# eovs/ldpc-lib

Hardware: AMD Instinct MI355X
Metric: decoded frames/sec, (2048,1024) QC-LDPC, 50 iters min-sum (higher is better)
Workload: dtype f64

## Files before the change

ldpc-lib_amd/csrc/ldpc_spec.hpp:

```cpp
#pragma once

#ifndef __HIPCC_RTC__
#include <hip/hip_runtime.h>
#endif
#include "lche_table.hpp"

namespace ldpc_spec {

typedef unsigned int u32;
typedef unsigned long long u64;

struct SpecArgs {
    const double *llr;
    u32 *hard;
    int *iters;
    double *soft_out;
    int maxiter;
    double alpha;
    const u32 *stale;
    u32 *synd_out;
    const int *frame_idx;
    const double *ims_coef;
    double ims_thr;
    int ims_max_quant, ims_max_data, ims_ialpha;
// ... 64 lines not shown
    0x0000000000000000ull, 0x3ff0000000000000ull, 0x3c9b3b4f1a88bf6eull, 0x3feff63da9fb3335ull,
    0xbc7160139cd8dc5dull, 0x3fefec9a3e778061ull, 0xbc905e7a108766d1ull, 0x3fefe315e86e7f85ull,
    0x3c8cd2523567f613ull, 0x3fefd9b0d3158574ull, 0xbc8bce8023f98efaull, 0x3fefd06b29ddf6deull,
    0x3c60f74e61e6c861ull, 0x3fefc74518759bc8ull, 0x3c90a3e45b33d399ull, 0x3fefbe3ecac6f383ull,
    0x3c979aa65d837b6dull, 0x3fefb5586cf9890full, 0x3c8eb51a92fdeffcull, 0x3fefac922b7247f7ull,
    0x3c3ebe3d702f9cd1ull, 0x3fefa3ec32d3d1a2ull, 0xbc6a033489906e0bull, 0x3fef9b66affed31bull,
    0xbc9556522a2fbd0eull, 0x3fef9301d0125b51ull, 0xbc5080ef8c4eea55ull, 0x3fef8abdc06c31ccull,
    0xbc91c923b9d5f416ull, 0x3fef829aaea92de0ull, 0x3c80d3e3e95c55afull, 0x3fef7a98c8a58e51ull,
    0xbc801b15eaa59348ull, 0x3fef72b83c7d517bull, 0xbc8f1ff055de323dull, 0x3fef6af9388c8deaull,
    0x3c8b898c3f1353bfull, 0x3fef635beb6fcb75ull, 0xbc96d99c7611eb26ull, 0x3fef5be084045cd4ull,
    0x3c9aecf73e3a2f60ull, 0x3fef54873168b9aaull, 0xbc8fe782cb86389dull, 0x3fef4d5022fcd91dull,
    0x3c8a6f4144a6c38dull, 0x3fef463b88628cd6ull, 0x3c807a05b0e4047dull, 0x3fef3f49917ddc96ull,
    0x3c968efde3a8a894ull, 0x3fef387a6e756238ull, 0x3c875e18f274487dull, 0x3fef31ce4fb2a63full,
    0x3c80472b981fe7f2ull, 0x3fef2b4565e27cddull, 0xbc96b87b3f71085eull, 0x3fef24dfe1f56381ull,
    0x3c82f7e16d09ab31ull, 0x3fef1e9df51fdee1ull, 0xbc3d219b1a6fbffaull, 0x3fef187fd0dad990ull,
    0x3c8b3782720c0ab4ull, 0x3fef1285a6e4030bull, 0x3c6e149289cecb8full, 0x3fef0cafa93e2f56ull,
    0x3c834d754db0abb6ull, 0x3fef06fe0a31b715ull, 0x3c864201e2ac744cull, 0x3fef0170fc4cd831ull,
    0x3c8fdd395dd3f84aull, 0x3feefc08b26416ffull, 0xbc86a3803b8e5b04ull, 0x3feef6c55f929ff1ull,
    0xbc924aedcc4b5068ull, 0x3feef1a7373aa9cbull, 0xbc9907f81b512d8eull, 0x3feeecae6d05d866ull,
    0xbc71d1e83e9436d2ull, 0x3feee7db34e59ff7ull, 0xbc991919b3ce1b15ull, 0x3feee32dc313a8e5ull,
    0x3c859f48a72a4c6dull, 0x3feedea64c123422ull, 0xbc9312607a28698aull, 0x3feeda4504ac801cull,
    0xbc58a78f4817895bull, 0x3feed60a21f72e2aull, 0xbc7c2c9b67499a1bull, 0x3feed1f5d950a897ull,
    0x3c4363ed60c2ac11ull, 0x3feece086061892dull, 0x3c9666093b0664efull, 0x3feeca41ed1d0057ull,
    0x3c6ecce1daa10379ull, 0x3feec6a2b5c13cd0ull, 0x3c93ff8e3f0f1230ull, 0x3feec32af0d7d3deull,
    0x3c7690cebb7aafb0ull, 0x3feebfdad5362a27ull, 0x3c931dbdeb54e077ull, 0x3feebcb299fddd0dull,
    0xbc8f94340071a38eull, 0x3feeb9b2769d2ca7ull, 0xbc87deccdc93a349ull, 0x3feeb6daa2cf6642ull,
    0xbc78dec6bd0f385full, 0x3feeb42b569d4f82ull, 0xbc861246ec7b5cf6ull, 0x3feeb1a4ca5d920full,
    0x3c93350518fdd78eull, 0x3feeaf4736b527daull, 0x3c7b98b72f8a9b05ull, 0x3feead12d497c7fdull,
    0x3c9063e1e21c5409ull, 0x3feeab07dd485429ull, 0x3c34c7855019c6eaull, 0x3feea9268a5946b7ull,
    0x3c9432e62b64c035ull, 0x3feea76f15ad2148ull, 0xbc8ce44a6199769full, 0x3feea5e1b976dc09ull,
    0xbc8c33c53bef4da8ull, 0x3feea47eb03a5585ull, 0xbc845378892be9aeull, 0x3feea34634ccc320ull,
    0xbc93cedd78565858ull, 0x3feea23882552225ull, 0x3c5710aa807e1964ull, 0x3feea155d44ca973ull,
    0xbc93b3efbf5e2228ull, 0x3feea09e667f3bcdull, 0xbc6a12ad8734b982ull, 0x3feea012750bdabfull,
    0xbc6367efb86da9eeull, 0x3fee9fb23c651a2full, 0xbc80dc3d54e08851ull, 0x3fee9f7df9519484ull,
    0xbc781f647e5a3ecfull, 0x3fee9f75e8ec5f74ull, 0xbc86ee4ac08b7db0ull, 0x3fee9f9a48a58174ull,
    0xbc8619321e55e68aull, 0x3fee9feb564267c9ull, 0x3c909ccb5e09d4d3ull, 0x3feea0694fde5d3full,
    0xbc7b32dcb94da51dull, 0x3feea11473eb0187ull, 0x3c94ecfd5467c06bull, 0x3feea1ed0130c132ull,
    0x3c65ebe1abd66c55ull, 0x3feea2f336cf4e62ull, 0xbc88a1c52fb3cf42ull, 0x3feea427543e1a12ull,
    0xbc9369b6f13b3734ull, 0x3feea589994cce13ull, 0xbc805e843a19ff1eull, 0x3feea71a4623c7adull,
    0xbc94d450d872576eull, 0x3feea8d99b4492edull, 0x3c90ad675b0e8a00ull, 0x3feeaac7d98a6699ull,
    0x3c8db72fc1f0eab4ull, 0x3feeace5422aa0dbull, 0xbc65b6609cc5e7ffull, 0x3feeaf3216b5448cull,
    0x3c7bf68359f35f44ull, 0x3feeb1ae99157736ull, 0xbc93091fa71e3d83ull, 0x3feeb45b0b91ffc6ull,
    0xbc5da9b88b6c1e29ull, 0x3feeb737b0cdc5e5ull, 0xbc6c23f97c90b959ull, 0x3feeba44cbc8520full,
    0xbc92434322f4f9aaull, 0x3feebd829fde4e50ull, 0xbc85ca6cd7668e4bull, 0x3feec0f170ca07baull,
    0x3c71affc2b91ce27ull, 0x3feec49182a3f090ull, 0x3c6dd235e10a73bbull, 0x3feec86319e32323ull,
    0xbc87c50422622263ull, 0x3feecc667b5de565ull, 0x3c8b1c86e3e231d5ull, 0x3feed09bec4a2d33ull,
    0xbc91bbd1d3bcbb15ull, 0x3feed503b23e255dull, 0x3c90cc319cee31d2ull, 0x3feed99e1330b358ull,
    0x3c8469846e735ab3ull, 0x3feede6b5579fdbfull, 0xbc82dfcd978e9db4ull, 0x3feee36bbfd3f37aull,
    0x3c8c1a7792cb3387ull, 0x3feee89f995ad3adull, 0xbc907b8f4ad1d9faull, 0x3feeee07298db666ull,
    0xbc55c3d956dcaebaull, 0x3feef3a2b84f15fbull, 0xbc90a40e3da6f640ull, 0x3feef9728de5593aull,
    0xbc68d6f438ad9334ull, 0x3feeff76f2fb5e47ull, 0xbc91eee26b588a35ull, 0x3fef05b030a1064aull,
    0x3c74ffd70a5fddcdull, 0x3fef0c1e904bc1d2ull, 0xbc91bdfbfa9298acull, 0x3fef12c25bd71e09ull,
    0x3c736eae30af0cb3ull, 0x3fef199bdd85529cull, 0x3c8ee3325c9ffd94ull, 0x3fef20ab5fffd07aull,
    0x3c84e08fd10959acull, 0x3fef27f12e57d14bull, 0x3c63cdaf384e1a67ull, 0x3fef2f6d9406e7b5ull,
    0x3c676b2c6c921968ull, 0x3fef3720dcef9069ull, 0xbc808a1883ccb5d2ull, 0x3fef3f0b555dc3faull,
    0xbc8fad5d3ffffa6full, 0x3fef472d4a07897cull, 0xbc900dae3875a949ull, 0x3fef4f87080d89f2ull,
    0x3c74a385a63d07a7ull, 0x3fef5818dcfba487ull, 0xbc82919e2040220full, 0x3fef60e316c98398ull,
    0x3c8e5a50d5c192acull, 0x3fef69e603db3285ull, 0x3c843a59ac016b4bull, 0x3fef7321f301b460ull,
    0xbc82d52107b43e1full, 0x3fef7c97337b9b5full, 0xbc892ab93b470dc9ull, 0x3fef864614f5a129ull,
    0x3c74b604603a88d3ull, 0x3fef902ee78b3ff6ull, 0x3c83c5ec519d7271ull, 0x3fef9a51fbc74c83ull,
    0xbc8ff7128fd391f0ull, 0x3fefa4afa2a490daull, 0xbc8dae98e223747dull, 0x3fefaf482d8e67f1ull,
    0x3c8ec3bc41aa2008ull, 0x3fefba1bee615a27ull, 0x3c842b94c3a9eb32ull, 0x3fefc52b376bba97ull,
    0x3c8a64a931d185eeull, 0x3fefd0765b6e4540ull, 0xbc8e37bae43be3edull, 0x3fefdbfdad9cbe14ull,
    0x3c77893b4d91cd9dull, 0x3fefe7c1819e90d8ull, 0x3c5305c14160cc89ull, 0x3feff3c22b8f71f1ull
};
template <class Tab>
__device__ __forceinline__ double exp_glibc_t(double x, Tab T) {
    const double InvLn2N = 0x1.71547652b82fep+7, Shift = 0x1.8p52, NegLn2hiN = -0x1.62e42fefa0000p-8, NegLn2loN = -0x1.cf79abc9e3b3ap-47;
    const double C2 = 0x1.ffffffffffdbdp-2, C3 = 0x1.555555555543cp-3, C4 = 0x1.55555cf172b91p-5, C5 = 0x1.1111167a4d017p-7;
    const double z = InvLn2N * x;
    double kd = z + Shift;
    const unsigned long long ki = (unsigned long long)__double_as_longlong(kd);
    kd -= Shift;
    const double r = __fma_rn(kd, NegLn2loN, __fma_rn(kd, NegLn2hiN, x));
    const unsigned long long idx = 2 * (ki % 128);
    const ulonglong2 pair = *reinterpret_cast<const ulonglong2 *>(&T[idx]);
    const double tail = __longlong_as_double((long long)pair.x);
    const unsigned long long sbits = pair.y + (ki << (52 - 7));
    const double r2 = r * r;
    const double tmp = __fma_rn(r2 * r2, __fma_rn(r, C5, C4), __fma_rn(r2, __fma_rn(r, C3, C2), tail + r));
    const double scale = __longlong_as_double((long long)sbits);
    return __fma_rn(scale, tmp, scale);
}
__device__ __forceinline__ double exp_glibc(double x) { return exp_glibc_t(x, kExpTab); }

__device__ __attribute__((aligned(16))) const unsigned long long kLogData[274] = {
    0x3fe62e42fefa3800ull, 0x3d2ef35793c76730ull, 0xbfe0000000000001ull, 0x3fd555555551305bull,
    0xbfcfffffffeb4590ull, 0x3fc999b324f10111ull, 0xbfc55575e506c89full, 0xbfe0000000000000ull,
    0x3fd5555555555577ull, 0xbfcffffffffffdcbull, 0x3fc999999995dd0cull, 0xbfc55555556745a7ull,
    0x3fc24924a344de30ull, 0xbfbfffffa4423d65ull, 0x3fbc7184282ad6caull, 0xbfb999eb43b068ffull,
    0x3fb78182f7afd085ull, 0xbfb5521375d145cdull, 0x3ff734f0c3e0de9full, 0xbfd7cc7f79e69000ull,
    0x3ff713786a2ce91full, 0xbfd76feec20d0000ull, 0x3ff6f26008fab5a0ull, 0xbfd713e31351e000ull,
    0x3ff6d1a61f138c7dull, 0xbfd6b85b38287800ull, 0x3ff6b1490bc5b4d1ull, 0xbfd65d5590807800ull,
    0x3ff69147332f0cbaull, 0xbfd602d076180000ull, 0x3ff6719f18224223ull, 0xbfd5a8ca86909000ull,
    0x3ff6524f99a51ed9ull, 0xbfd54f4356035000ull, 0x3ff63356aa8f24c4ull, 0xbfd4f637c36b4000ull,
    0x3ff614b36b9ddc14ull, 0xbfd49da7fda85000ull, 0x3ff5f66452c65c4cull, 0xbfd445923989a800ull,
    0x3ff5d867b5912c4full, 0xbfd3edf439b0b800ull, 0x3ff5babccb5b90deull, 0xbfd396ce448f7000ull,
    0x3ff59d61f2d91a78ull, 0xbfd3401e17bda000ull, 0x3ff5805612465687ull, 0xbfd2e9e2ef468000ull,
    0x3ff56397cee76bd3ull, 0xbfd2941b3830e000ull, 0x3ff54725e2a77f93ull, 0xbfd23ec58cda8800ull,
    0x3ff52aff42064583ull, 0xbfd1e9e129279000ull, 0x3ff50f22dbb2bddfull, 0xbfd1956d2b48f800ull,
    0x3ff4f38f4734ded7ull, 0xbfd141679ab9f800ull, 0x3ff4d843cfde2840ull, 0xbfd0edd094ef9800ull,
    0x3ff4bd3ec078a3c8ull, 0xbfd09aa518db1000ull, 0x3ff4a27fc3e0258aull, 0xbfd047e65263b800ull,
    0x3ff4880524d48434ull, 0xbfcfeb224586f000ull, 0x3ff46dce1b192d0bull, 0xbfcf474a7517b000ull,
    0x3ff453d9d3391854ull, 0xbfcea4443d103000ull, 0x3ff43a2744b4845aull, 0xbfce020d44e9b000ull,
    0x3ff420b54115f8fbull, 0xbfcd60a22977f000ull, 0x3ff40782da3ef4b1ull, 0xbfccc00104959000ull,
    0x3ff3ee8f5d57fe8full, 0xbfcc202956891000ull, 0x3ff3d5d9a00b4ce9ull, 0xbfcb81178d811000ull,
    0x3ff3bd60c010c12bull, 0xbfcae2c9ccd3d000ull, 0x3ff3a5242b75dab8ull, 0xbfca45402e129000ull,
    0x3ff38d22cd9fd002ull, 0xbfc9a877681df000ull, 0x3ff3755bc5847a1cull, 0xbfc90c6d69483000ull,
    0x3ff35dce49ad36e2ull, 0xbfc87120a645c000ull, 0x3ff34679984dd440ull, 0xbfc7d68fb4143000ull,
    0x3ff32f5cceffcb24ull, 0xbfc73cb83c627000ull, 0x3ff3187775a10d49ull, 0xbfc6a39a9b376000ull,
    0x3ff301c8373e3990ull, 0xbfc60b3154b7a000ull, 0x3ff2eb4ebb95f841ull, 0xbfc5737d76243000ull,
    0x3ff2d50a0219a9d1ull, 0xbfc4dc7b8fc23000ull, 0x3ff2bef9a8b7fd2aull, 0xbfc4462c51d20000ull,
    0x3ff2a91c7a0c1babull, 0xbfc3b08abc830000ull, 0x3ff293726014b530ull, 0xbfc31b996b490000ull,
    0x3ff27dfa5757a1f5ull, 0xbfc2875490a44000ull, 0x3ff268b39b1d3bbfull, 0xbfc1f3b9f879a000ull,
    0x3ff2539d838ff5bdull, 0xbfc160c8252ca000ull, 0x3ff23eb7aac9083bull, 0xbfc0ce7f57f72000ull,
    0x3ff22a012ba940b6ull, 0xbfc03cdc49fea000ull, 0x3ff2157996cc4132ull, 0xbfbf57bdbc4b8000ull,
    0x3ff201201dd2fc9bull, 0xbfbe370896404000ull, 0x3ff1ecf4494d480bull, 0xbfbd17983ef94000ull,
    0x3ff1d8f5528f6569ull, 0xbfbbf9674ed8a000ull, 0x3ff1c52311577e7cull, 0xbfbadc79202f6000ull,
    0x3ff1b17c74cb26e9ull, 0xbfb9c0c3e7288000ull, 0x3ff19e010c2c1ab6ull, 0xbfb8a646b372c000ull,
    0x3ff18ab07bb670bdull, 0xbfb78d01b3ac0000ull, 0x3ff1778a25efbcb6ull, 0xbfb674f145380000ull,
    0x3ff1648d354c31daull, 0xbfb55e0e6d878000ull, 0x3ff151b990275fddull, 0xbfb4485cdea1e000ull,
    0x3ff13f0ea432d24cull, 0xbfb333d94d6aa000ull, 0x3ff12c8b7210f9daull, 0xbfb22079f8c56000ull,
    0x3ff11a3028ecb531ull, 0xbfb10e4698622000ull, 0x3ff107fbda8434afull, 0xbfaffa6c6ad20000ull,
    0x3ff0f5ee0f4e6bb3ull, 0xbfadda8d4a774000ull, 0x3ff0e4065d2a9fceull, 0xbfabbcece4850000ull,
    0x3ff0d244632ca521ull, 0xbfa9a1894012c000ull, 0x3ff0c0a77ce2981aull, 0xbfa788583302c000ull,
    0x3ff0af2f83c636d1ull, 0xbfa5715e67d68000ull, 0x3ff09ddb98a01339ull, 0xbfa35c8a49658000ull,
    0x3ff08cabaf52e7dfull, 0xbfa149e364154000ull, 0x3ff07b9f2f4e28fbull, 0xbf9e72c082eb8000ull,
    0x3ff06ab58c358f19ull, 0xbf9a55f152528000ull, 0x3ff059eea5ecf92cull, 0xbf963d62cf818000ull,
    0x3ff04949cdd12c90ull, 0xbf9228fb8caa0000ull, 0x3ff038c6c6f0ada9ull, 0xbf8c317b20f90000ull,
    0x3ff02865137932a9ull, 0xbf8419355daa0000ull, 0x3ff0182427ea7348ull, 0xbf781203c2ec0000ull,
    0x3ff008040614b195ull, 0xbf60040979240000ull, 0x3fefe01ff726fa1aull, 0x3f6feff384900000ull,
    0x3fefa11cc261ea74ull, 0x3f87dc41353d0000ull, 0x3fef6310b081992eull, 0x3f93cea3c4c28000ull,
    0x3fef25f63ceeadcdull, 0x3f9b9fc114890000ull, 0x3feee9c8039113e7ull, 0x3fa1b0d8ce110000ull,
    0x3feeae8078cbb1abull, 0x3fa58a5bd001c000ull, 0x3fee741aa29d0c9bull, 0x3fa95c8340d88000ull,
    0x3fee3a91830a99b5ull, 0x3fad276aef578000ull, 0x3fee01e009609a56ull, 0x3fb07598e598c000ull,
    0x3fedca01e577bb98ull, 0x3fb253f5e30d2000ull, 0x3fed92f20b7c9103ull, 0x3fb42edd8b380000ull,
    0x3fed5cac66fb5cceull, 0x3fb606598757c000ull, 0x3fed272caa5ede9dull, 0x3fb7da76356a0000ull,
    0x3fecf26e3e6b2ccdull, 0x3fb9ab434e1c6000ull, 0x3fecbe6da2a77902ull, 0x3fbb78c7bb0d6000ull,
    0x3fec8b266d37086dull, 0x3fbd431332e72000ull, 0x3fec5894bd5d5804ull, 0x3fbf0a3171de6000ull,
    0x3fec26b533bb9f8cull, 0x3fc067152b914000ull, 0x3febf583eeece73full, 0x3fc147858292b000ull,
    0x3febc4fd75db96c1ull, 0x3fc2266ecdca3000ull, 0x3feb951e0c864a28ull, 0x3fc303d7a6c55000ull,
    0x3feb65e2c5ef3e2cull, 0x3fc3dfc33c331000ull, 0x3feb374867c9888bull, 0x3fc4ba366b7a8000ull,
    0x3feb094b211d304aull, 0x3fc5933928d1f000ull, 0x3feadbe885f2ef7eull, 0x3fc66acd2418f000ull,
    0x3feaaf1d31603da2ull, 0x3fc740f8ec669000ull, 0x3fea82e63fd358a7ull, 0x3fc815c0f51af000ull,
    0x3fea5740ef09738bull, 0x3fc8e92954f68000ull, 0x3fea2c2a90ab4b27ull, 0x3fc9bb3602f84000ull,
    0x3fea01a01393f2d1ull, 0x3fca8bed1c2c0000ull, 0x3fe9d79f24db3c1bull, 0x3fcb5b515c01d000ull,
    0x3fe9ae2505c7b190ull, 0x3fcc2967ccbcc000ull, 0x3fe9852ef297ce2full, 0x3fccf635d5486000ull,
    0x3fe95cbaeea44b75ull, 0x3fcdc1bd3446c000ull, 0x3fe934c69de74838ull, 0x3fce8c01b8cfe000ull,
    0x3fe90d4f2f6752e6ull, 0x3fcf5509c0179000ull, 0x3fe8e6528effd79dull, 0x3fd00e6c121fb800ull,
    0x3fe8bfce9fcc007cull, 0x3fd071b80e93d000ull, 0x3fe899c0dabec30eull, 0x3fd0d46b9e867000ull,
    0x3fe87427aa2317fbull, 0x3fd13687334bd000ull, 0x3fe84f00acb39a08ull, 0x3fd1980d67234800ull,
    0x3fe82a49e8653e55ull, 0x3fd1f8ffe0cc8000ull, 0x3fe8060195f40260ull, 0x3fd2595fd7636800ull,
    0x3fe7e22563e0a329ull, 0x3fd2b9300914a800ull, 0x3fe7beb377dcb5adull, 0x3fd3187210436000ull,
    0x3fe79baa679725c2ull, 0x3fd377266dec1800ull, 0x3fe77907f2170657ull, 0x3fd3d54ffbaf3000ull,
    0x3fe756cadbd6130cull, 0x3fd432eee32fe000ull
};
template <class Tab>
__device__ __forceinline__ double log_glibc_t(double x, Tab T) {
    auto D = [&](int i) { return __longlong_as_double((long long)kLogData[i]); };
    unsigned long long ix = (unsigned long long)__double_as_longlong(x);
    const u32 top = (u32)(ix >> 48);
    const unsigned long long LO = 0x3fee000000000000ull , HI = 0x3ff1090000000000ull ;
    if (ix - LO < HI - LO) {
        if (ix == 0x3ff0000000000000ull) return 0.0;
        const double r = x - 1.0, r2 = r * r, r3 = r * r2;
        const double t3 = __fma_rn(r3, D(17), __fma_rn(r2, D(16), __fma_rn(r, D(15), D(14))));
        const double t2 = __fma_rn(r3, t3, __fma_rn(r2, D(13), __fma_rn(r, D(12), D(11))));
        const double t1 = __fma_rn(r3, t2, __fma_rn(r2, D(10), __fma_rn(r, D(9), D(8))));
        double w = r * 0x1p27;
        const double rhi = r + w - w, rlo = r - rhi;
        w = rhi * rhi * D(7);
        const double hi = r + w;
        double lo = r - hi + w;
        lo = __fma_rn(D(7) * rlo, rhi + r, lo);
        return __fma_rn(t1, r3, lo) + hi;
    }
    if (top - 0x0010u >= 0x7ff0u - 0x0010u) {
        if (ix * 2 == 0) return -__longlong_as_double(0x7ff0000000000000ll);
        if (ix == 0x7ff0000000000000ull) return x;
        if ((top & 0x8000u) || (top & 0x7ff0u) == 0x7ff0u) return __longlong_as_double(0x7ff8000000000000ll) ;
        ix = (unsigned long long)__double_as_longlong(x * 0x1p52);
        ix -= 52ull << 52;
    }
    const unsigned long long tmp = ix - 0x3fe6000000000000ull;
    const int i = (int)((tmp >> (52 - 7)) % 128);
    const long long k = (long long)tmp >> 52;
    const unsigned long long iz = ix - (tmp & (0xfffull << 52));
    const ulonglong2 cpair = *reinterpret_cast<const ulonglong2 *>(&T[18 + 2 * i]);
    const double invc = __longlong_as_double((long long)cpair.x), logc = __longlong_as_double((long long)cpair.y), z = __longlong_as_double((long long)iz);
    const double r = __fma_rn(z, invc, -1.0);
    const double kd = (double)k;
    const double w = __fma_rn(kd, D(0), logc);
    const double hi = w + r;
    const double lo = __fma_rn(kd, D(1), w - hi + r);
    const double r2 = r * r;
    const double p = __fma_rn(r, D(6), D(5));
    const double q = __fma_rn(r2, p, __fma_rn(r, D(4), D(3)));
    return __fma_rn(r * r2, q, __fma_rn(r2, D(2), lo)) + hi;
}
__device__ __forceinline__ double log_glibc(double x) { return log_glibc_t(x, kLogData); }
template <class Tab>
__device__ __forceinline__ double exp_glibc_wide(double x, Tab T) {
    return fabs(x) < 512.0 ? exp_glibc_t(x, T) : exp(x);
}
constexpr int kBpTabWords = 256 + 274;

__device__ __forceinline__ double at_most(double x, double hi) { return fmin(x, hi); }
__device__ __forceinline__ double at_least(double x, double lo) { return fmax(x, lo); }

template <bool QUEUED, class F>
__device__ __forceinline__ void for_each_frame(const SpecArgs &a, long long fr, F body) {
    if constexpr (!QUEUED) {
        body(fr);
    } else {
        __shared__ unsigned q_ticket;
        while (fr < a.nframes) {
            body(fr);
            if (!a.queue) break;
            __syncthreads();
            if (threadIdx.x == 0) q_ticket = atomicAdd(a.queue, 1u);
            __syncthreads();
            fr = (long long)gridDim.x + (long long)(unsigned)__builtin_amdgcn_readfirstlane((int)q_ticket);
        }
    }
}

template <int N, int T, class Pred>
__device__ __forceinline__ void pack_hard(u32 *dst, const int tid, Pred pred) {
    constexpr int G = (N + 63) / 64, HW = (N + 31) / 32;
    const int lane = tid & 63;
    for (int g = tid >> 6; g < G; g += T / 64) {
        const int v = 64 * g + lane;
        const u64 m = __ballot(v < N && pred(v < N ? v : 0));
        if (lane == 0) {
            dst[2 * g] = (u32)m;
            if (2 * g + 1 < HW) dst[2 * g + 1] = (u32)(m >> 32);
        }
    }
}


constexpr unsigned long kMsM64LdsBytes(unsigned long n) { return sizeof(double) * n + 512; }

constexpr int kMsM64LocalSpan = 3;
template <class C>
constexpr int ms_m64_slot_of(int j, int k) {
    for (int s = 0; s < C::RW[j]; ++s)
        if (C::COL[j][s] == k) return s;
    return -1;
}
template <class C>
constexpr int ms_m64_first_row(int k) {
    for (int j = 0; j < C::RH; ++j)
        if (ms_m64_slot_of<C>(j, k) >= 0) return j;
    return -1;
}
template <class C>
constexpr int ms_m64_last_row(int k) {
    for (int j = C::RH - 1; j >= 0; --j)
        if (ms_m64_slot_of<C>(j, k) >= 0) return j;
    return -1;
}
template <class C>
constexpr bool ms_m64_local_col(int k) {
    for (int j = 0; j < C::RH; ++j) {
        const int s = ms_m64_slot_of<C>(j, k);
        if (s >= 0 && C::SH[j][s] != 0) return false;
    }
    return ms_m64_first_row<C>(k) >= 0 && ms_m64_last_row<C>(k) - ms_m64_first_row<C>(k) <= kMsM64LocalSpan;
}
template <class C>
constexpr int ms_m64_local_starts(int j) {
    int n = 0;
    for (int s = 0; j < C::RH && s < C::RW[j]; ++s)
        n += ms_m64_local_col<C>(C::COL[j][s]) && ms_m64_first_row<C>(C::COL[j][s]) == j ? 1 : 0;
    return n;
}
template <class C>
constexpr int ms_m64_row_edges(int j) {
    int n = 0;
    for (int s = 0; s < C::RW[j]; ++s) n += ms_m64_local_col<C>(C::COL[j][s]) ? 0 : 1;
    return n;
}

template <class C>
constexpr int ms_m64_keep_rows(int budget) {
    int edges = 0, rows = 0;
    while (rows < C::RH && 2 * (edges + ms_m64_row_edges<C>(rows)) - 5 * (rows + 1) <= budget) edges += ms_m64_row_edges<C>(rows++);
    return rows;
}
constexpr int kMsM64KeepEdges = 68, kMsM64KeepRowsOfExample = 13;
template <class C>
constexpr int ms_m64_keep_budget() {
    constexpr int cols = C::NH < 24 ? C::NH : 24;
    constexpr int others = 5 * C::RH + 2 * cols + 2 * C::WMAX, others_example = 5 * 16 + 2 * 24 + 2 * 8;
    constexpr int cut = others > others_example ? others - others_example : 0;
    constexpr int regs = 2 * kMsM64KeepEdges - 5 * kMsM64KeepRowsOfExample;
    return regs > cut ? regs - cut : 0;
}

template <int KPCAP>
constexpr int ms_m64_prefix_rows(int kr) { return KPCAP < kr ? (KPCAP > 0 ? KPCAP : 0) : kr; }

template <class C, int KPCAP = 1 << 30>
__device__ __forceinline__ void ms_m64_body(const SpecArgs &a) {
    static_assert(C::M == 64, "ms_m64_body: one frame per wavefront needs M == 64");
    constexpr int RH = C::RH, NH = C::NH, N = C::NH * 64;
    constexpr int KR = ms_m64_keep_rows<C>(ms_m64_keep_budget<C>());
    typedef IC<ms_m64_prefix_rows<KPCAP>(KR)> KP;
    extern __shared__ double lds[];
    const int lane = threadIdx.x;
    const double alpha = a.alpha, alpha_mag = fabs(a.alpha);
    long long fr = blockIdx.x;

    const u32 lane8 = (u32)lane * 8u;
    const u32 lo = lds_addr(lds) + lane8, hi = lo + 512u;
    auto at = [&](u32 tie, auto S, auto K) -> double * {
        constexpr int c = decltype(S)::value, k = decltype(K)::value;
        static_assert(c >= 0 && c < 64 && k * 512 + c * 8 < 65536, "shift / block column out of range");
        if constexpr (c == 0) return lds_at(hi + (u32)(k * 512));
        else return lds_at(sel32_tied(hi, lo, ~0ull << (64 - c), tie) + (u32)(k * 512 + c * 8));
    };
    auto own = [&](auto K) -> double * { return lds_at(hi + (u32)(decltype(K)::value * 512)); };

  while (fr < a.nframes) {
    const double *const yrow = a.llr + fr * N + lane;
    const __amdgpu_buffer_rsrc_t ybuf = __builtin_amdgcn_make_buffer_rsrc(const_cast<double *>(a.llr + fr * N), 0, N * 8, 0x00020000);

    double m1[RH], m2[RH];
    u32 meta[RH];
    double keep[RH][C::WMAX];
    static_for<0, RH>([&](auto J) {
        constexpr int j = decltype(J)::value;
        m1[j] = 0.0; m2[j] = 0.0; meta[j] = 0u;
        if constexpr (j < KR) static_for<0, C::RW[j]>([&](auto S) { keep[j][decltype(S)::value] = 0.0; });
    });

    int res = -a.maxiter;
    for (int iter = 0; iter < a.maxiter; ++iter) {
        double y[NH];
        auto load_y = [&](auto K0, auto K1) {
            int yo = 0;
            asm volatile("" : "+v"(yo));
            static_for<decltype(K0)::value, (decltype(K1)::value < NH ? decltype(K1)::value : NH)>([&](auto K) {
                constexpr int k = decltype(K)::value;
                if constexpr (!ms_m64_local_col<C>(k)) y[k] = yrow[yo + k * 64];
            });
        };
        double yl[NH], soft_l[NH];
        auto load_yl = [&](auto JN) {
            constexpr int jn = decltype(JN)::value;
            if constexpr (ms_m64_local_starts<C>(jn) > 0) {
                u32 so = 0;
                asm volatile("" : "+s"(so));
                static_for<0, C::RW[jn]>([&](auto S) {
                    constexpr int k = C::COL[jn][decltype(S)::value];
                    if constexpr (ms_m64_local_col<C>(k) && ms_m64_first_row<C>(k) == jn) {
                        typedef u32 u32x2 __attribute__((ext_vector_type(2)));
                        const u32x2 v = __builtin_amdgcn_raw_buffer_load_b64(ybuf, (int)lane8, (int)(so + (u32)(k * 512)), 0);
                        yl[k] = mk(v.y, v.x);
                    }
                });
            }
        };
        static_for<0, RH>([&](auto J) {
            constexpr int j = decltype(J)::value;
            if constexpr (j < KR) {
                u32 tie;
                asm volatile("" : "=v"(tie));
                static_for<0, C::RW[j]>([&](auto S) {
                    constexpr int s = decltype(S)::value;
                    if constexpr (!ms_m64_local_col<C>(C::COL[j][s])) {
                        const double cv = keep[j][s];
                        double *p = at(tie, IC<C::SH[j][s]>{}, IC<C::COL[j][s]>{});
                        if constexpr (C::FIRST[j][s]) *p = cv;
                        else __hip_atomic_fetch_add(p, cv, __ATOMIC_RELAXED, __HIP_MEMORY_SCOPE_WORKGROUP);
                    }
                });
            } else {
                u32 mt = meta[j];
                asm volatile("" : "+v"(mt));
                const u32 pos = mt & 0xffu;
                u32 Wt = mt;
                static_for<0, C::RW[j]>([&](auto S) {
                    constexpr int s = decltype(S)::value;
                    if constexpr (ms_m64_local_col<C>(C::COL[j][s])) {
                        Wt = twice(Wt);
                    } else {
                        const double aa = sel64(m1[j], m2[j], lanes_eq(pos, (u32)s));
                        const double cv = signed_mag(aa, Wt);
                        Wt = twice(Wt);
                        double *p = at(mt, IC<C::SH[j][s]>{}, IC<C::COL[j][s]>{});
                        if constexpr (C::FIRST[j][s]) *p = cv;
                        else __hip_atomic_fetch_add(p, cv, __ATOMIC_RELAXED, __HIP_MEMORY_SCOPE_WORKGROUP);
                    }
                });
            }
            __builtin_amdgcn_sched_barrier(0);
        });
        load_y(IC<0>{}, IC<16>{});
        static_for<0, NH>([&](auto K) {
            constexpr int k = decltype(K)::value;
            if constexpr (k % 8 == 0 && k + 16 < NH) load_y(IC<k + 16>{}, IC<k + 24>{});
            if constexpr (!ms_m64_local_col<C>(k)) {
                double *p = own(K);
                const double pr = *p * alpha;
                *p = (y[k] + 0.0) + pr;
            }
            if constexpr (k % 8 == 7) __builtin_amdgcn_sched_barrier(0);
        });
        load_yl(IC<0>{});
        u32 failw = 0;
        static_for<0, RH>([&](auto J) {
            constexpr int j = decltype(J)::value;
            constexpr int RW = C::RW[j];
            u32 mt = meta[j];
            asm volatile("" : "+v"(mt));
            load_yl(IC<j + 1>{});
            double nm1 = kMaxVal, nm2 = kMaxVal;
            u32 npos = 0, nS = 0, sy = 0;
            double r[RW], tt_[RW];
            static_for<0, RW>([&](auto S) {
                constexpr int s = decltype(S)::value;
                constexpr int k = C::COL[j][s];
                if constexpr (!ms_m64_local_col<C>(k)) {
                    r[s] = *at(mt, IC<C::SH[j][s]>{}, IC<k>{});
                } else {
                    if constexpr (ms_m64_first_row<C>(k) == j) {
                        double acc = 0.0;
                        static_for<j, ms_m64_last_row<C>(k) + 1>([&](auto JJ) {
                            constexpr int jj = decltype(JJ)::value, ss = ms_m64_slot_of<C>(jj, k);
                            if constexpr (ss >= 0) {
                                if constexpr (jj >= KR) {
                                    const u32 m = jj == j ? mt : meta[jj];
                                    const double aa = sel64(m1[jj], m2[jj], lanes_eq(m & 0xffu, (u32)ss));
                                    keep[jj][ss] = signed_mag(aa, ss == 0 ? m : ss == 1 ? twice(m) : m << ss);
                                }
                                const double cv = keep[jj][ss];
                                if constexpr (jj == j) acc = cv;
                                else acc = acc + cv;
                            }
                        });
                        const double pr = acc * alpha;
                        soft_l[k] = (yl[k] + 0.0) + pr;
                        *own(IC<k>{}) = soft_l[k];
                    }
                    r[s] = soft_l[k];
                }
            });
            auto step = [&](auto S, double x) {
                constexpr int s = decltype(S)::value;
                const double tt = r[s] - x;
                nS = __builtin_amdgcn_alignbit(nS, hi32(tt), 31);
                const double v = fabs(tt);
                if constexpr (j < KR) tt_[s] = tt;
                if constexpr (s == 0) {
                    nm1 = fmin(v, kMaxVal);
                } else if constexpr (j < KR) {
                    nm2 = fmin(fmax(v, nm1), nm2);
                    nm1 = fmin(v, nm1);
                } else {
                    const mask64 c1 = lanes_lt(v, nm1);
                    nm2 = fmin(fmax(v, nm1), nm2);
                    npos = sel32(npos, (u32)s, c1);
                    nm1 = fmin(v, nm1);
                }
            };
            if constexpr (j < KR) {
                if constexpr (j < KP::value) {
                    double pf[RW > 1 ? RW - 1 : 1];
                    static_for<0, RW>([&](auto S) {
                        constexpr int s = decltype(S)::value;
                        sy ^= hi32(r[s]);
                        const double tt = r[s] - keep[j][s] * alpha_mag;
                        nS ^= hi32(tt);
                        tt_[s] = tt;
                        if constexpr (s == 0 && RW > 1) pf[0] = fmin(fabs(tt), kMaxVal);
                        else if constexpr (s > 0 && s < RW - 1) pf[s] = fmin(fabs(tt), pf[s - 1]);
                    });
                    double suf = kMaxVal;
                    static_for<0, RW>([&](auto S) {
                        constexpr int s = RW - 1 - decltype(S)::value;
                        double mag;
                        if constexpr (RW == 1) mag = kMaxVal;
                        else if constexpr (s == RW - 1) mag = pf[RW - 2];
                        else if constexpr (s == 0) mag = suf;
                        else mag = fmin(pf[s - 1], suf);
                        if constexpr (s > 0) suf = fmin(fabs(tt_[s]), suf);
                        keep[j][s] = signed_mag(mag, hi32(tt_[s]) ^ nS);
                    });
                } else {
                    static_for<0, RW>([&](auto S) {
                        constexpr int s = decltype(S)::value;
                        sy ^= hi32(r[s]);
                        step(S, keep[j][s] * alpha_mag);
                    });
                }
            } else {
                const u32 pos = mt & 0xffu;
                u32 Wt = mt;
                double a1 = m1[j] * alpha, a2 = m2[j] * alpha;
                asm volatile("" : "+v"(a1), "+v"(a2));
                static_for<0, RW>([&](auto S) {
                    constexpr int s = decltype(S)::value;
                    sy ^= hi32(r[s]);
                    if constexpr (ms_m64_local_col<C>(C::COL[j][s])) {
                        Wt = twice(Wt);
                        step(S, keep[j][s] * alpha_mag);
                    } else {
                        const double aa = sel64(a1, a2, lanes_eq(pos, (u32)s));
                        const double x = signed_mag(aa, Wt);
                        Wt = twice(Wt);
                        step(S, x);
                    }
                });
            }
            failw |= sy;
            asm volatile("" : "+v"(failw));
            if constexpr (j < KR) {
                if constexpr (j >= KP::value) {
                    u32 W = (nS ^ (0u - (__popc(nS) & 1u))) << (32 - RW);
                    static_for<0, RW>([&](auto S) {
                        constexpr int s = decltype(S)::value;
                        keep[j][s] = signed_mag(sel64(nm1, nm2, lanes_oeq(fabs(tt_[s]), nm1)), W);
                        W = twice(W);
                    });
                }
            } else {
                m1[j] = nm1; m2[j] = nm2; meta[j] = ((nS ^ (0u - (__popc(nS) & 1u))) << (32 - RW)) | npos;
            }
            __builtin_amdgcn_sched_barrier(0);
        });
        if (__ballot((failw >> 31) != 0) == 0ull) { res = iter + 1; break; }
    }

    if (lane == 0 && a.iters) a.iters[fr] = res;
    if (a.hard) {
        u64 mine = 0ull;
        static_for<0, NH>([&](auto K) {
            constexpr int k = decltype(K)::value;
            const u64 b = __ballot((hi32(*own(K)) >> 31) != 0);
            if (lane == k) mine = b;
        });
        if (lane < NH) reinterpret_cast<u64 *>(a.hard + fr * (N / 32))[lane] = mine;
    }
    if (a.soft_out) {
        static_for<0, NH>([&](auto K) {
            constexpr int k = decltype(K)::value;
            a.soft_out[fr * N + k * 64 + lane] = *own(K);
        });
    }
    if (!a.queue) break;
    u32 ticket = 0;
    if (lane == 0) ticket = atomicAdd(a.queue, 1u);
    fr = (long long)gridDim.x + (long long)(u32)__builtin_amdgcn_readfirstlane((int)ticket);
  }
}

template <class C>
__device__ __forceinline__ void ms_body(const SpecArgs &a) {
    constexpr int RH = C::RH, NH = C::NH, M = C::M, N = NH * M, W = (M + 63) / 64;
    constexpr bool POW2 = (M & (M - 1)) == 0;
    extern __shared__ double lds[];
    char *const ldsb = reinterpret_cast<char *>(lds);
    int *const flag = reinterpret_cast<int *>(ldsb + (size_t)N * 8);
    const int n = threadIdx.x;
    const bool valid = (M % 64 == 0) || n < M;
    const u32 n8 = (u32)(valid ? n : 0) * 8u;
    const double alpha = a.alpha;
    for_each_frame<true>(a, (long long)blockIdx.x, [&](const long long fr) {

    auto rot = [&](u32 base, auto S) -> u32 {
        constexpr int c = decltype(S)::value;
        if constexpr (c == 0) return base;
        else if constexpr (POW2) return (base + 8u * (u32)c) & (u32)(8 * M - 1);
        else { const u32 t = base + 8u * (u32)c, w = t - (u32)(8 * M); return t < w ? t : w; }
    };
    FrameVote fvote;
    if constexpr (W > 1) fvote.init(flag);
    auto vote = [&](bool fail) -> bool {
        if constexpr (W == 1) return __ballot(fail) != 0ull;
        else return fvote(fail);
    };
    const double *const yrow = a.llr + fr * N + (valid ? n : 0);

    double m1[RH], m2[RH];
    u32 meta[RH];
    static_for<0, RH>([&](auto J) { constexpr int j = decltype(J)::value; m1[j] = 0.0; m2[j] = 0.0; meta[j] = 0u; });

    int res = -a.maxiter;
    for (int iter = 0; iter < a.maxiter; ++iter) {
        double y[NH];
        int yo = 0;
        asm volatile("" : "+v"(yo));
        static_for<0, NH>([&](auto K) { constexpr int k = decltype(K)::value; y[k] = yrow[yo + k * M]; });
        static_for<0, RH>([&](auto J) {
            constexpr int j = decltype(J)::value;
            u32 mt = meta[j], nb = n8;
            asm volatile("" : "+v"(mt), "+v"(nb) :: "memory");
            const u32 pos = mt & 0xffu;
            u32 Wt = mt;
            static_for<0, C::RW[j]>([&](auto S) {
                constexpr int s = decltype(S)::value;
                const double aa = sel64(m1[j], m2[j], lanes_eq(pos, (u32)s));
                const double cv = signed_mag(aa, Wt);
                Wt = twice(Wt);
                double *p = reinterpret_cast<double *>(ldsb + rot(nb, IC<C::SH[j][s]>{}) + C::COL[j][s] * (8 * M));
                if (valid) {
                    if constexpr (C::FIRST[j][s]) *p = cv;
                    else __hip_atomic_fetch_add(p, cv, __ATOMIC_RELAXED, __HIP_MEMORY_SCOPE_WORKGROUP);
                }
            });
            if constexpr (W > 1) __syncthreads();
            else __builtin_amdgcn_sched_barrier(0);
        });
        if (valid) {
            static_for<0, NH>([&](auto K) {
                constexpr int k = decltype(K)::value;
                double *p = reinterpret_cast<double *>(ldsb + n8 + k * (8 * M));
                const double pr = *p * alpha;
                *p = (y[k] + 0.0) + pr;
                if constexpr (k % 8 == 7) __builtin_amdgcn_sched_barrier(0);
            });
        }
        if constexpr (W > 1) __syncthreads();
        u32 failw = 0;
        static_for<0, RH>([&](auto J) {
            constexpr int j = decltype(J)::value;
            constexpr int RW = C::RW[j];
            u32 mt = meta[j];
            asm volatile("" : "+v"(mt) :: "memory");
            const u32 pos = mt & 0xffu;
            u32 Wt = mt;
            double a1 = m1[j] * alpha, a2 = m2[j] * alpha;
            asm volatile("" : "+v"(a1), "+v"(a2));
            double nm1 = kMaxVal, nm2 = kMaxVal;
            u32 npos = 0, nS = 0, sy = 0;
            u32 nb = n8;
            asm volatile("" : "+v"(nb));
            double r[RW];
            static_for<0, RW>([&](auto S) {
                constexpr int s = decltype(S)::value;
                r[s] = *reinterpret_cast<const double *>(ldsb + rot(nb, IC<C::SH[j][s]>{}) + C::COL[j][s] * (8 * M));
            });
            static_for<0, RW>([&](auto S) {
                constexpr int s = decltype(S)::value;
                sy ^= hi32(r[s]);
                const double aa = sel64(a1, a2, lanes_eq(pos, (u32)s));
                const double x = signed_mag(aa, Wt);
                Wt = twice(Wt);
                const double tt = r[s] - x;
                nS = __builtin_amdgcn_alignbit(nS, hi32(tt), 31);
                const double v = fabs(tt);
                const mask64 c1 = lanes_lt(v, nm1);
                nm2 = fmin(fmax(v, nm1), nm2);
                npos = sel32(npos, (u32)s, c1);
                nm1 = fmin(v, nm1);
            });
            failw |= sy;
            m1[j] = nm1; m2[j] = nm2; meta[j] = ((nS ^ (0u - (__popc(nS) & 1u))) << (32 - RW)) | npos;
            asm volatile("" : "+v"(m1[j]), "+v"(m2[j]), "+v"(meta[j]));
            __builtin_amdgcn_sched_barrier(0);
        });
        if (!vote(valid && (failw >> 31) != 0)) { res = iter + 1; break; }
    }

    if (threadIdx.x == 0 && a.iters) a.iters[fr] = res;
    if (a.hard) {
        constexpr int HW = (N + 31) / 32;
        if constexpr (M % 64 == 0) {
            const int wave = threadIdx.x >> 6, lane = threadIdx.x & 63;
            static_for<0, NH>([&](auto K) {
                constexpr int k = decltype(K)::value;
                const u64 b = __ballot((*reinterpret_cast<const u32 *>(ldsb + n8 + k * (8 * M) + 4) >> 31) != 0);
                if (lane == 0) reinterpret_cast<u64 *>(a.hard + fr * HW)[k * W + wave] = b;
            });
        } else {
            pack_hard<N, W * 64>(a.hard + fr * HW, threadIdx.x, [&](int v) { return (*reinterpret_cast<const u32 *>(ldsb + (size_t)v * 8 + 4) >> 31) != 0; });
        }
    }
    if (a.soft_out && valid) {
        static_for<0, NH>([&](auto K) {
            constexpr int k = decltype(K)::value;
            a.soft_out[fr * N + k * M + n] = *reinterpret_cast<const double *>(ldsb + n8 + k * (8 * M));
        });
    }
    });
}

template <class C>
__device__ __forceinline__ void ms_small_body(const SpecArgs &a) {
    constexpr int RH = C::RH, NH = C::NH, M = C::M, N = NH * M, F = 64 / M;
    static_assert(M <= 32 && F >= 2, "ms_small_body: M <= 32");
    constexpr bool POW2 = (M & (M - 1)) == 0;
    extern __shared__ double lds[];
    const int lane = threadIdx.x;
    const int f = lane / M, n = lane - f * M;
    const long long fr = (long long)blockIdx.x * F + f;
    const bool live = f < F && fr < a.nframes;
    char *const ldsb = reinterpret_cast<char *>(lds) + (size_t)(live ? f : 0) * N * 8;
    const u32 n8 = (u32)n * 8u;
    const double alpha = a.alpha;
    const u64 frame_lanes = (M == 32 ? 0xffffffffull : ((1ull << M) - 1ull)) << ((live ? f : 0) * M);

    auto rot = [&](u32 base, auto S) -> u32 {
        constexpr int c = decltype(S)::value;
        if constexpr (c == 0) return base;
        else if constexpr (POW2) return (base + 8u * (u32)c) & (u32)(8 * M - 1);
        else { const u32 t = base + 8u * (u32)c, w = t - (u32)(8 * M); return t < w ? t : w; }
    };
    const double *const yrow = a.llr + (live ? fr : 0) * N + n;

    double m1[RH], m2[RH];
    u32 meta[RH];
    static_for<0, RH>([&](auto J) { constexpr int j = decltype(J)::value; m1[j] = 0.0; m2[j] = 0.0; meta[j] = 0u; });

    bool done = !live;
    int res = -a.maxiter;
    for (int iter = 0; iter < a.maxiter; ++iter) {
        double y[NH];
        int yo = 0;
        asm volatile("" : "+v"(yo));
        static_for<0, NH>([&](auto K) { constexpr int k = decltype(K)::value; y[k] = yrow[yo + k * M]; });
        if (!done) static_for<0, RH>([&](auto J) {
            constexpr int j = decltype(J)::value;
            u32 mt = meta[j], nb = n8;
            asm volatile("" : "+v"(mt), "+v"(nb));
            const u32 pos = mt & 0xffu;
            u32 Wt = mt;
            static_for<0, C::RW[j]>([&](auto S) {
                constexpr int s = decltype(S)::value;
                const double aa = sel64(m1[j], m2[j], lanes_eq(pos, (u32)s));
                const double cv = signed_mag(aa, Wt);
                Wt = twice(Wt);
                double *p = reinterpret_cast<double *>(ldsb + rot(nb, IC<C::SH[j][s]>{}) + C::COL[j][s] * (8 * M));
                if constexpr (C::FIRST[j][s]) *p = cv;
                else __hip_atomic_fetch_add(p, cv, __ATOMIC_RELAXED, __HIP_MEMORY_SCOPE_WORKGROUP);
            });
            __builtin_amdgcn_sched_barrier(0);
        });
        asm volatile("" ::: "memory");
        if (!done) {
            static_for<0, NH>([&](auto K) {
                constexpr int k = decltype(K)::value;
                double *p = reinterpret_cast<double *>(ldsb + n8 + k * (8 * M));
                const double pr = *p * alpha;
                *p = (y[k] + 0.0) + pr;
                if constexpr (k % 8 == 7) __builtin_amdgcn_sched_barrier(0);
            });
        }
        asm volatile("" ::: "memory");
        u32 failw = 0;
        if (!done) static_for<0, RH>([&](auto J) {
            constexpr int j = decltype(J)::value;
            constexpr int RW = C::RW[j];
            u32 mt = meta[j];
            asm volatile("" : "+v"(mt));
            const u32 pos = mt & 0xffu;
            u32 Wt = mt;
            double a1 = m1[j] * alpha, a2 = m2[j] * alpha;
            asm volatile("" : "+v"(a1), "+v"(a2));
            double nm1 = kMaxVal, nm2 = kMaxVal;
            u32 npos = 0, nS = 0, sy = 0;
            u32 nb = n8;
            asm volatile("" : "+v"(nb));
            double r[RW];
            static_for<0, RW>([&](auto S) {
                constexpr int s = decltype(S)::value;
                r[s] = *reinterpret_cast<const double *>(ldsb + rot(nb, IC<C::SH[j][s]>{}) + C::COL[j][s] * (8 * M));
            });
            static_for<0, RW>([&](auto S) {
                constexpr int s = decltype(S)::value;
                sy ^= hi32(r[s]);
                const double aa = sel64(a1, a2, lanes_eq(pos, (u32)s));
                const double x = signed_mag(aa, Wt);
                Wt = twice(Wt);
                const double tt = r[s] - x;
                nS = __builtin_amdgcn_alignbit(nS, hi32(tt), 31);
                const double v = fabs(tt);
                const mask64 c1 = lanes_lt(v, nm1);
                nm2 = fmin(fmax(v, nm1), nm2);
                npos = sel32(npos, (u32)s, c1);
                nm1 = fmin(v, nm1);
            });
            failw |= sy;
            m1[j] = nm1; m2[j] = nm2; meta[j] = ((nS ^ (0u - (__popc(nS) & 1u))) << (32 - RW)) | npos;
            asm volatile("" : "+v"(m1[j]), "+v"(m2[j]), "+v"(meta[j]));
            __builtin_amdgcn_sched_barrier(0);
        });
        asm volatile("" ::: "memory");
        const u64 failing = __ballot(!done && (failw >> 31) != 0);
        if (!done && (failing & frame_lanes) == 0ull) { done = true; res = iter + 1; }
        if (__ballot(!done) == 0ull) break;
    }

    if (!live) return;
    if (n == 0 && a.iters) a.iters[fr] = res;
    if (a.hard) {
        constexpr int HW = (N + 31) / 32;
        for (int w = n; w < HW; w += M) {
            u32 bits = 0;
            for (int b = 0; b < 32; ++b) {
                const int v = 32 * w + b;
                if (v < N) bits |= (*reinterpret_cast<const u32 *>(ldsb + (size_t)v * 8 + 4) >> 31) << b;
            }
            a.hard[fr * HW + w] = bits;
        }
    }
    if (a.soft_out) {
        static_for<0, NH>([&](auto K) {
            constexpr int k = decltype(K)::value;
            a.soft_out[fr * N + k * M + n] = *reinterpret_cast<const double *>(ldsb + n8 + k * (8 * M));
        });
    }
}

template <class C>
__device__ __forceinline__ void ms_chunk_body(const SpecArgs &a) {
    constexpr int RH = C::RH, NH = C::NH, M = C::M, N = NH * M, CH = (M + 63) / 64;
    static_assert(M > 64 && CH == 2, "ms_chunk_body: 64 < M <= 128");
    constexpr bool POW2 = (M & (M - 1)) == 0;
    extern __shared__ double lds[];
    char *const ldsb = reinterpret_cast<char *>(lds);
    const int lane = threadIdx.x;
    const double alpha = a.alpha;
    for_each_frame<true>(a, (long long)blockIdx.x, [&](const long long fr) {
    bool ok[CH];
    u32 n8[CH];
    static_for<0, CH>([&](auto Q) {
        constexpr int ch = decltype(Q)::value;
        ok[ch] = (64 * ch + 64 <= M) || (64 * ch + lane < M);
        n8[ch] = (u32)(ok[ch] ? 64 * ch + lane : 0) * 8u;
    });
    auto rot = [&](u32 base, auto S) -> u32 {
        constexpr int c = decltype(S)::value;
        if constexpr (c == 0) return base;
        else if constexpr (POW2) return (base + 8u * (u32)c) & (u32)(8 * M - 1);
        else { const u32 t = base + 8u * (u32)c, w = t - (u32)(8 * M); return t < w ? t : w; }
    };

    double m1[CH][RH], m2[CH][RH];
    u32 meta[CH][RH];
    static_for<0, CH>([&](auto Q) {
        static_for<0, RH>([&](auto J) {
            constexpr int ch = decltype(Q)::value, j = decltype(J)::value;
            m1[ch][j] = 0.0; m2[ch][j] = 0.0; meta[ch][j] = 0u;
        });
    });

    int res = -a.maxiter;
    for (int iter = 0; iter < a.maxiter; ++iter) {
        static_for<0, RH>([&](auto J) {
// ... 1538 lines not shown
```

Baseline: 6.189 million.

## Shallow buffer-load prefetch of channel LLRs and spend freed registers on kept rows

Replaces the 16-to-24-column-ahead global loads of the channel LLRs with raw buffer loads over only the non-local columns, prefetching a configurable depth (default 8) and optionally issuing them inside a chosen check-row. The registers no longer held by in-flight loads are counted at compile time and used to keep more check rows' messages in registers (a larger KR), capped by a register budget. This is meant to cut LDS message reconstruction work and shorten live ranges, but shallower prefetch can expose more memory latency and the higher register count risks spills.

```diff
diff --git a/ldpc-lib_amd/csrc/ldpc_spec.hpp b/ldpc-lib_amd/csrc/ldpc_spec.hpp
--- a/ldpc-lib_amd/csrc/ldpc_spec.hpp
+++ b/ldpc-lib_amd/csrc/ldpc_spec.hpp
@@ -390,11 +390,52 @@
 template <int KPCAP>
 constexpr int ms_m64_prefix_rows(int kr) { return KPCAP < kr ? (KPCAP > 0 ? KPCAP : 0) : kr; }
 
-template <class C, int KPCAP = 1 << 30>
+template <class C>
+constexpr int ms_m64_nonlocal_cols() {
+    int n = 0;
+    for (int k = 0; k < C::NH; ++k) n += ms_m64_local_col<C>(k) ? 0 : 1;
+    return n;
+}
+template <class C>
+constexpr int ms_m64_nonlocal_col(int n) {
+    for (int k = 0; k < C::NH; ++k)
+        if (!ms_m64_local_col<C>(k) && n-- == 0) return k;
+    return -1;
+}
+constexpr int kMsM64YDepth = 8;
+template <class C>
+constexpr int ms_m64_y_in_flight_r23() {
+    int peak = 0;
+    for (int k0 = 0; k0 < C::NH; k0 += 8) {
+        int n = 0;
+        for (int k = k0; k < C::NH && k < k0 + 24; ++k) n += ms_m64_local_col<C>(k) ? 0 : 1;
+        peak = n > peak ? n : peak;
+    }
+    return peak;
+}
+constexpr int kMsM64State3Regs = 244;
+template <class C>
+constexpr int ms_m64_state3_regs(int rows) {
+    int e = 0;
+    for (int j = 0; j < rows; ++j) e += C::RW[j];
+    return 2 * e + 5 * (C::RH - rows) + 4 * C::WMAX - 2;
+}
+template <class C, int YD>
+constexpr int ms_m64_carry_rows() {
+    constexpr int nl = ms_m64_nonlocal_cols<C>(), depth = YD < nl ? YD : nl, was = ms_m64_y_in_flight_r23<C>();
+    constexpr int base = ms_m64_keep_rows<C>(ms_m64_keep_budget<C>());
+    constexpr int more = base > 0 ? ms_m64_keep_rows<C>(ms_m64_keep_budget<C>() + 2 * (was > depth ? was - depth : 0)) : 0;
+    int rows = base;
+    while (rows < more && ms_m64_state3_regs<C>(rows + 1) <= kMsM64State3Regs) ++rows;
+    return rows;
+}
+
+template <class C, int KPCAP = 1 << 30, int YD = kMsM64YDepth, int YROW = -1, int KRSET = -1>
 __device__ __forceinline__ void ms_m64_body(const SpecArgs &a) {
     static_assert(C::M == 64, "ms_m64_body: one frame per wavefront needs M == 64");
+    static_assert(YD >= 1 && YROW >= -1 && YROW < C::RH && KRSET <= C::RH, "ms_m64_body: switch out of range");
     constexpr int RH = C::RH, NH = C::NH, N = C::NH * 64;
-    constexpr int KR = ms_m64_keep_rows<C>(ms_m64_keep_budget<C>());
+    constexpr int KR = KRSET >= 0 ? KRSET : ms_m64_carry_rows<C, YD>();
     typedef IC<ms_m64_prefix_rows<KPCAP>(KR)> KP;
     extern __shared__ double lds[];
     const int lane = threadIdx.x;
@@ -412,7 +453,6 @@
     auto own = [&](auto K) -> double * { return lds_at(hi + (u32)(decltype(K)::value * 512)); };
 
   while (fr < a.nframes) {
-    const double *const yrow = a.llr + fr * N + lane;
     const __amdgpu_buffer_rsrc_t ybuf = __builtin_amdgcn_make_buffer_rsrc(const_cast<double *>(a.llr + fr * N), 0, N * 8, 0x00020000);
 
     double m1[RH], m2[RH];
@@ -426,14 +466,19 @@
 
     int res = -a.maxiter;
     for (int iter = 0; iter < a.maxiter; ++iter) {
+        constexpr int NL = ms_m64_nonlocal_cols<C>(), YAHEAD = YD < NL ? YD : NL;
         double y[NH];
-        auto load_y = [&](auto K0, auto K1) {
-            int yo = 0;
-            asm volatile("" : "+v"(yo));
-            static_for<decltype(K0)::value, (decltype(K1)::value < NH ? decltype(K1)::value : NH)>([&](auto K) {
-                constexpr int k = decltype(K)::value;
-                if constexpr (!ms_m64_local_col<C>(k)) y[k] = yrow[yo + k * 64];
-            });
+        auto load_y = [&](auto N0, auto N1) {
+            if constexpr (decltype(N0)::value < NL && decltype(N0)::value < decltype(N1)::value) {
+u32 so = 0;
+                asm volatile("" : "+s"(so));
+                static_for<decltype(N0)::value, (decltype(N1)::value < NL ? decltype(N1)::value : NL)>([&](auto I) {
+                    constexpr int k = ms_m64_nonlocal_col<C>(decltype(I)::value);
+                    typedef u32 u32x2 __attribute__((ext_vector_type(2)));
+                    const u32x2 v = __builtin_amdgcn_raw_buffer_load_b64(ybuf, (int)lane8, (int)(so + (u32)(k * 512)), 0);
+                    y[k] = mk(v.y, v.x);
+                });
+            }
         };
         double yl[NH], soft_l[NH];
         auto load_yl = [&](auto JN) {
@@ -485,17 +530,19 @@
                 });
             }
             __builtin_amdgcn_sched_barrier(0);
-        });
-        load_y(IC<0>{}, IC<16>{});
-        static_for<0, NH>([&](auto K) {
-            constexpr int k = decltype(K)::value;
-            if constexpr (k % 8 == 0 && k + 16 < NH) load_y(IC<k + 16>{}, IC<k + 24>{});
-            if constexpr (!ms_m64_local_col<C>(k)) {
-                double *p = own(K);
-                const double pr = *p * alpha;
-                *p = (y[k] + 0.0) + pr;
+            if constexpr (j == YROW) {
+                load_y(IC<0>{}, IC<YAHEAD>{});
+                __builtin_amdgcn_sched_barrier(0);
             }
-            if constexpr (k % 8 == 7) __builtin_amdgcn_sched_barrier(0);
+        });
+        if constexpr (YROW < 0) load_y(IC<0>{}, IC<YAHEAD>{});
+        static_for<0, NL>([&](auto I) {
+            constexpr int i = decltype(I)::value, k = ms_m64_nonlocal_col<C>(i);
+            if constexpr (i % 2 == 0) load_y(IC<i + YAHEAD>{}, IC<i + YAHEAD + 2>{});
+            double *p = own(IC<k>{});
+            const double pr = *p * alpha;
+            *p = (y[k] + 0.0) + pr;
+            if constexpr (i % 2 == 1) __builtin_amdgcn_sched_barrier(0);
         });
         load_yl(IC<0>{});
         u32 failw = 0;
@@ -622,20 +669,22 @@
         if (__ballot((failw >> 31) != 0) == 0ull) { res = iter + 1; break; }
     }
 
+    int ol = lane;
+    if constexpr (KR > 0) asm volatile("" : "+v"(ol));
     if (lane == 0 && a.iters) a.iters[fr] = res;
     if (a.hard) {
         u64 mine = 0ull;
         static_for<0, NH>([&](auto K) {
             constexpr int k = decltype(K)::value;
             const u64 b = __ballot((hi32(*own(K)) >> 31) != 0);
-            if (lane == k) mine = b;
-        });
-        if (lane < NH) reinterpret_cast<u64 *>(a.hard + fr * (N / 32))[lane] = mine;
+            if (ol == k) mine = b;
+        });
+        if (ol < NH) reinterpret_cast<u64 *>(a.hard + fr * (N / 32))[ol] = mine;
     }
     if (a.soft_out) {
         static_for<0, NH>([&](auto K) {
             constexpr int k = decltype(K)::value;
-            a.soft_out[fr * N + k * 64 + lane] = *own(K);
+            a.soft_out[fr * N + k * 64 + ol] = *own(K);
         });
     }
     if (!a.queue) break;
```

New measurement: 6.423 million (median of 6 runs). 1.04x the previous value.
